# COMPiLELab/krylov_robustness

Measured on NVIDIA B200. Metric: krylov_matvecs_per_sec, higher is better.
Workload: dtype f64

## Files before the change

krylov_robustness_b200/csrc/api.cu:

```cuda
#include <memory>
#include <thread>
#include "common.cuh"
#include "csr.cuh"
#include "spmm.cuh"
#include "dense.cuh"
#include "slq.cuh"
#include "theta_table.h"
#include "smalldense.cuh"
#include "pairs.cuh"
#include "pairs_small.cuh"
#include "expmv.cuh"
#include "tsdense.cuh"
#include "smallgemm.cuh"
#include "vecops.cuh"
#include "blockkrylov.cuh"
#include "entries.cuh"
#include "entries_local.cuh"
#include "frechet.cuh"
#include "mctrace.cuh"
#include "nodepairs.cuh"

using namespace kr;

static void destroy_fun_update_result(kr_ctx* c);
// ... 15 lines not shown
        cudaError_t e = cudaGetDeviceCount(&count);
        if (e != cudaSuccess || count == 0) {
            cudaGetLastError();
            fail(KR_ERR_CUDA, "no CUDA device available (%s); this library has no CPU fallback",
                 e == cudaSuccess ? "device count is 0" : cudaGetErrorString(e));
        }
        if (device < 0 || device >= count) fail(KR_ERR_ARG, "device %d out of range (0..%d)", device, count - 1);
        KR_CUDA(cudaSetDevice(device));
        cudaDeviceProp prop;
        KR_CUDA(cudaGetDeviceProperties(&prop, device));
        if (prop.major < 10)
            fail(KR_ERR_CUDA, "device %d is sm_%d%d; this library is built for sm_100a only", device,
                 prop.major, prop.minor);
        kr_ctx* c = new kr_ctx();
        c->device = device;
        c->num_sms = prop.multiProcessorCount;
        c->l2_bytes = (size_t)prop.l2CacheSize;
        KR_CUDA(cudaStreamCreateWithFlags(&c->stream, cudaStreamNonBlocking));
        *out = c;
    });
}

void kr_ctx_destroy(kr_ctx* c) {
    if (!c) return;
    cudaSetDevice(c->device);
    cudaStreamSynchronize(c->stream);
    destroy_fun_update_result(c);
    for (auto& ev : c->spmm_events) {
        cudaEventDestroy(ev.first);
        cudaEventDestroy(ev.second);
    }
    for (auto ev : c->free_events) cudaEventDestroy(ev);
    c->trim();
    if (c->copy_stream) cudaStreamDestroy(c->copy_stream);
    if (c->stream) cudaStreamDestroy(c->stream);
    delete c;
}

int kr_ctx_sync(kr_ctx* c) {
    return guarded([&] {
        KR_CUDA(cudaSetDevice(c->device));
        KR_CUDA(cudaStreamSynchronize(c->stream));
    });
}

int kr_ctx_counters(kr_ctx* c, int64_t out[5]) {
    return guarded([&] {
        for (int i = 0; i < 5; ++i) out[i] = c->counters[i];
    });
}

int kr_ctx_set_timing(kr_ctx* c, int on) {
    return guarded([&] { c->timing = on != 0; });
}

int kr_ctx_spmm_time(kr_ctx* c, int reset, double* ms, int64_t* launches) {
    return guarded([&] {
        KR_CUDA(cudaStreamSynchronize(c->stream));
        for (auto& ev : c->spmm_events) {
            float t = 0.f;
            KR_CUDA(cudaEventElapsedTime(&t, ev.first, ev.second));
            c->spmm_ms += t;
            c->spmm_timed += 1;
            c->free_events.push_back(ev.first);
            c->free_events.push_back(ev.second);
        }
        c->spmm_events.clear();
        if (ms) *ms = c->spmm_ms;
        if (launches) *launches = c->spmm_timed;
        if (reset) {
            c->spmm_ms = 0.0;
            c->spmm_timed = 0;
        }
    });
}

void* kr_ctx_stream(kr_ctx* c) { return c ? (void*)c->stream : nullptr; }

int kr_matrix_create(kr_ctx* ctx, int64_t n, int64_t nnz, const int64_t* row_ptr, const int64_t* col_idx,
                     const double* val, kr_matrix** out) {
    return guarded([&] {
        if (!ctx || !out || !row_ptr || (nnz > 0 && (!col_idx || !val)))
            fail(KR_ERR_ARG, "kr_matrix_create: null argument");
        if (n < 0 || nnz < 0 || row_ptr[0] != 0 || row_ptr[n] != nnz)
            fail(KR_ERR_ARG, "kr_matrix_create: inconsistent row_ptr (the matrix A should be square, CSR, 0-based)");
        KR_CUDA(cudaSetDevice(ctx->device));
        std::unique_ptr<kr_matrix> M(new kr_matrix());
        M->ctx = ctx;
        M->host.n = n;
        M->host.row_ptr.assign(row_ptr, row_ptr + n + 1);
        M->host.col.resize(nnz);
        M->host.val.resize(nnz);
        for (int64_t i = 0; i < n; ++i)
            if (row_ptr[i + 1] < row_ptr[i]) fail(KR_ERR_ARG, "kr_matrix_create: row_ptr not monotone");
        int bad = 0;
#pragma omp parallel for reduction(|| : bad) schedule(static)
        for (int64_t p = 0; p < nnz; ++p) {
            bad = bad || col_idx[p] < 0 || col_idx[p] >= n;
            M->host.col[p] = (int32_t)col_idx[p];
            M->host.val[p] = val[p];
        }
        if (bad) fail(KR_ERR_ARG, "kr_matrix_create: column index out of range (The matrix A should be square)");
        analyse_and_upload(M.get());
        *out = M.release();
        if (const char* e = getenv("KR_GPUS")) {
            const int want = atoi(e);
            if (want > 1 && kr_matrix_replicate(*out, want, nullptr) != 0) {
                const std::string m = kr_last_error();
                kr_matrix_destroy(*out);
                *out = nullptr;
                fail(KR_ERR_CUDA, "KR_GPUS=%d: %s", want, m.c_str());
            }
        }
    });
}

void kr_matrix_destroy(kr_matrix* A) {
    if (!A) return;
    for (kr_matrix* P : A->peers) {
        kr_ctx* pc = P->ctx;
        cudaSetDevice(pc->device);
        delete P;
        kr_ctx_destroy(pc);
    }
    A->peers.clear();
    cudaSetDevice(A->ctx->device);
    delete A;
}

int kr_matrix_replicate(kr_matrix* A, int ndev, const int* devices) {
    return guarded([&] {
        if (!A || A->is_peer) fail(KR_ERR_ARG, "kr_matrix_replicate: null matrix or a replica");
        if (!A->peers.empty()) fail(KR_ERR_ARG, "kr_matrix_replicate: the matrix already has replicas");
        int count = 0;
        KR_CUDA(cudaGetDeviceCount(&count));
        std::vector<int> devs;
        if (ndev <= 0 || !devices) {
            const int want = ndev <= 0 ? count : std::min(ndev, count);
            for (int d = 0; d < count && (int)devs.size() < want - 1; ++d)
                if (d != A->ctx->device) devs.push_back(d);
        } else {
            for (int k = 0; k < ndev; ++k) {
                if (devices[k] < 0 || devices[k] >= count) fail(KR_ERR_ARG, "kr_matrix_replicate: device %d out of range", devices[k]);
                if (devices[k] != A->ctx->device) devs.push_back(devices[k]);
            }
        }
        materialize(A);
        const CsrHost& H = A->host;
        std::vector<int> status(devs.size(), 0);
        std::vector<std::string> msg(devs.size());
        std::vector<kr_matrix*> made(devs.size(), nullptr);
        std::vector<std::thread> th;
        for (size_t k = 0; k < devs.size(); ++k)
            th.emplace_back([&, k] {
                status[k] = guarded([&] {
                    kr_ctx* pc = nullptr;
                    if (kr_ctx_create(devs[k], &pc) != 0) fail(KR_ERR_CUDA, "%s", kr_last_error());
                    std::unique_ptr<kr_matrix> M(new kr_matrix());
                    M->ctx = pc;
                    M->host = H;
                    M->is_peer = true;
                    try { analyse_and_upload(M.get()); } catch (...) { M.reset(); kr_ctx_destroy(pc); throw; }
                    made[k] = M.release();
                });
                if (status[k]) msg[k] = kr_last_error();
            });
        for (auto& t : th) t.join();
        for (size_t k = 0; k < devs.size(); ++k)
            if (status[k]) {
                for (kr_matrix* P : made)
                    if (P) { kr_ctx* pc = P->ctx; cudaSetDevice(pc->device); delete P; kr_ctx_destroy(pc); }
                fail(status[k], "%s", msg[k].c_str());
            }
        A->peers = made;
        KR_CUDA(cudaSetDevice(A->ctx->device));
    });
}

int kr_matrix_replicas(const kr_matrix* A) { return A ? 1 + (int)A->peers.size() : 0; }

int kr_matrix_info(const kr_matrix* A, int64_t* n, int64_t* nnz, int* symmetric, int* pattern_only,
                   int* nonnegative) {
    return guarded([&] {
        if (!A) fail(KR_ERR_ARG, "null matrix");
        if (n) *n = A->dev.n;
        if (nnz) *nnz = A->dev.nnz;
        if (symmetric) *symmetric = A->symmetric;
        if (pattern_only) *pattern_only = A->dev.pattern_only;
        if (nonnegative) *nonnegative = A->nonnegative;
    });
}

int kr_matrix_set_edges(kr_matrix* A, int64_t count, const int64_t* ii, const int64_t* jj, const double* v) {
    return guarded([&] {
        if (!A) fail(KR_ERR_ARG, "null matrix");
        KR_CUDA(cudaSetDevice(A->ctx->device));
        const CsrHost& H = A->host;
        const int64_t n = H.n;
        for (int64_t e = 0; e < count; ++e) {
            const int64_t i = ii[e] - 1, j = jj[e] - 1;
            if (i < 0 || i >= n || j < 0 || j >= n) fail(KR_ERR_ARG, "kr_matrix_set_edges: index out of range");
            A->pending[{i, j}] = v[e] - host_entry(H, i, j);
            A->pending[{j, i}] = v[e] - host_entry(H, j, i);
        }
        for (auto it = A->pending.begin(); it != A->pending.end();)
            it = (it->second == 0.0) ? A->pending.erase(it) : std::next(it);
        if (!A->symmetric || A->pending.size() > KR_MAX_PENDING) flush_pending(A);
        else upload_pending(A);
        for (kr_matrix* P : A->peers)
            if (kr_matrix_set_edges(P, count, ii, jj, v) != 0) fail(KR_ERR_CUDA, "replica on device %d: %s", P->ctx->device, kr_last_error());
        KR_CUDA(cudaSetDevice(A->ctx->device));
    });
}

int kr_dense_create(kr_ctx* ctx, int64_t n, int64_t k, kr_dense** out) {
    return guarded([&] {
        if (!ctx || !out || n < 0 || k < 0 || k > (1 << 20)) fail(KR_ERR_ARG, "kr_dense_create: bad argument");
        KR_CUDA(cudaSetDevice(ctx->device));
        std::unique_ptr<kr_dense> d(new kr_dense());
        d->ctx = ctx;
        d->buf.reset(ctx, n, (int)k);
        *out = d.release();
    });
}

void kr_dense_destroy(kr_dense* d) {
    if (!d) return;
    cudaSetDevice(d->ctx->device);
    delete d;
}

static void upload_cm(kr_ctx* ctx, const double* host, int64_t ld, PanelBuf& dst) { upload_cm_block(ctx, host, ld, dst); }
static void download_cm(kr_ctx* ctx, const PanelBuf& src, double* host, int64_t ld) { download_cm_block(ctx, src, host, ld); }

int kr_dense_upload(kr_dense* d, const double* host, int64_t ld) {
    return guarded([&] {
        if (!d || !host) fail(KR_ERR_ARG, "kr_dense_upload: null argument");
        KR_CUDA(cudaSetDevice(d->ctx->device));
        upload_cm(d->ctx, host, ld, d->buf);
    });
}

int kr_dense_download(const kr_dense* d, double* host, int64_t ld) {
    return guarded([&] {
        if (!d || !host) fail(KR_ERR_ARG, "kr_dense_download: null argument");
        KR_CUDA(cudaSetDevice(d->ctx->device));
        download_cm(d->ctx, d->buf, host, ld);
    });
}

int kr_dense_fill_rademacher(kr_dense* d, uint64_t seed, int64_t col_offset) {
    return guarded([&] {
        if (!d) fail(KR_ERR_ARG, "null block");
        KR_CUDA(cudaSetDevice(d->ctx->device));
        if (d->buf.elems() == 0) return;
        KR_LAUNCH(d->ctx, rademacher_kernel, d->ctx->num_sms * 8, 256, 0, d->buf.p(), d->buf.n, d->buf.cols,
                  d->buf.panels, seed, col_offset);
    });
}

int kr_spmm_dev(kr_ctx* ctx, const kr_matrix* A, const kr_dense* X, kr_dense* Y) {
    return guarded([&] {
        if (!ctx || !A || !X || !Y) fail(KR_ERR_ARG, "kr_spmm_dev: null argument");
        if (X->buf.n != A->dev.n) fail(KR_ERR_ARG, "The block vector b has wrong number of rows");
        if (Y->buf.n != X->buf.n || Y->buf.cols != X->buf.cols || Y->buf.p() == X->buf.p())
            fail(KR_ERR_ARG, "kr_spmm_dev: Y must be a distinct block of the same shape as X");
        KR_CUDA(cudaSetDevice(ctx->device));
        EpiPlain epi{Y->buf.p(), X->buf.p(), 1.0, 0.0};
        launch_spmm(ctx, A->dev, X->buf.p(), X->buf.panels, epi, nullptr, X->buf.cols);
    });
}

int kr_spmm(kr_ctx* ctx, const kr_matrix* A, int64_t k, const double* X, int64_t ldx, double* Y, int64_t ldy) {
    return guarded([&] {
        if (!ctx || !A || !X || !Y) fail(KR_ERR_ARG, "kr_spmm: null argument");
        KR_CUDA(cudaSetDevice(ctx->device));
        const int64_t n = A->dev.n;
        PanelBuf xb(ctx, n, (int)k), yb(ctx, n, (int)k);
        upload_cm(ctx, X, ldx, xb);
        EpiPlain epi{yb.p(), xb.p(), 1.0, 0.0};
        launch_spmm(ctx, A->dev, xb.p(), xb.panels, epi, nullptr, (int)k);
        download_cm(ctx, yb, Y, ldy);
    });
}

static void slq_finish(const SlqResult& R, int64_t m, double* tr, double* vals, double* alpha, double* beta) {
    if (tr) *tr = R.tr;
    const size_t k = R.vals.size();
    if (vals) std::memcpy(vals, R.vals.data(), k * sizeof(double));
    if (alpha || beta)
        for (int64_t j = 0; j < m; ++j)
            for (size_t c = 0; c < k; ++c) {
                if (alpha) alpha[c * m + j] = R.alpha[(size_t)j * k + c];
                if (beta) beta[c * m + j] = R.beta[(size_t)j * k + c];
            }
}

int kr_slq_trace_dev(kr_ctx* ctx, const kr_matrix* A, const kr_dense* Z, int64_t m, int fun, double* tr,
                     double* vals, double* alpha, double* beta) {
    return guarded([&] {
        if (!ctx || !A || !Z) fail(KR_ERR_ARG, "kr_slq_trace_dev: null argument");
        if (fun < 0 || fun > 2) fail(KR_ERR_ARG, "unsupported function selector");
        KR_CUDA(cudaSetDevice(ctx->device));
        PanelBuf W(ctx, Z->buf.n, Z->buf.cols);
        KR_CUDA(cudaMemcpyAsync(W.p(), Z->buf.p(), (size_t)W.elems() * sizeof(double), cudaMemcpyDeviceToDevice,
                                ctx->stream));
        SlqResult R = slq_run(ctx, A, W, (int)m, fun, alpha || beta);
        slq_finish(R, m, tr, vals, alpha, beta);
    });
}

}

template <class T>
static int slq_trace_host(kr_ctx* ctx, const kr_matrix* A, int64_t k, const T* Z, int64_t ldz, int64_t m, int fun,
                          double* tr, double* vals, double* alpha, double* beta) {
    return guarded([&] {
        if (!ctx || !A || !Z) fail(KR_ERR_ARG, "kr_slq_trace: null argument");
        if (fun < 0 || fun > 2) fail(KR_ERR_ARG, "unsupported function selector");
        KR_CUDA(cudaSetDevice(ctx->device));
        const int64_t n = A->dev.n;
        if (ldz < n) fail(KR_ERR_ARG, "The block vector b has wrong number of rows");
        if (k <= 0) fail(KR_ERR_ARG, "kr_slq_trace: no probe columns");
        std::vector<int64_t> cstart, cwidth;
        for (int64_t c0 = 0; c0 < k;) {
            const int64_t cw = std::min<int64_t>(k - c0, cstart.empty() ? 2 * PW : (cstart.size() == 1 ? 6 * PW : 8 * PW));
            cstart.push_back(c0);
            cwidth.push_back(cw);
            c0 += cw;
        }
        if (cstart.empty()) { cstart.push_back(0); cwidth.push_back(0); }
        const int64_t nch = (int64_t)cstart.size();
        if (!ctx->copy_stream) KR_CUDA(cudaStreamCreateWithFlags(&ctx->copy_stream, cudaStreamNonBlocking));
        std::vector<std::unique_ptr<PanelBuf>> W(nch);
        std::vector<std::unique_ptr<DevBuf<T>>> stage(nch);
        std::vector<cudaEvent_t> ready(nch, nullptr);
        for (int64_t c = 0; c < nch; ++c) {
            W[c].reset(new PanelBuf(ctx, n, (int)cwidth[c]));
            stage[c].reset(new DevBuf<T>(ctx, (size_t)std::max<int64_t>(n * cwidth[c], 1)));
        }
        KR_CUDA(cudaStreamSynchronize(ctx->stream));
        auto issue_copy = [&](int64_t c) {
            const int64_t c0 = cstart[c], cw = cwidth[c];
            if (n > 0 && cw > 0) {
                KR_CUDA(cudaMemcpy2DAsync(stage[c]->p, n * sizeof(T), Z + c0 * ldz, ldz * sizeof(T),
                                          n * sizeof(T), cw, cudaMemcpyHostToDevice, ctx->copy_stream));
                ctx->counters[3] += n * cw * (int64_t)sizeof(T);
            }
            cm_to_panel(ctx, stage[c]->p, n, *W[c], ctx->copy_stream);
            KR_CUDA(cudaEventCreateWithFlags(&ready[c], cudaEventDisableTiming));
            KR_CUDA(cudaEventRecord(ready[c], ctx->copy_stream));
        };
        std::vector<double> all_vals((size_t)k), all_a, all_b;
        if (alpha || beta) { all_a.resize((size_t)m * k); all_b.resize((size_t)m * k); }
        auto harvest = [&](int64_t c, SlqJob& job) {
            const int64_t c0 = cstart[c], cw = cwidth[c];
            SlqResult R = job.collect();
            for (int64_t q = 0; q < cw; ++q) all_vals[(size_t)(c0 + q)] = R.vals[(size_t)q];
            if (alpha || beta)
                for (int64_t j = 0; j < m; ++j)
                    for (int64_t q = 0; q < cw; ++q) {
                        all_a[(size_t)(j * k + c0 + q)] = R.alpha[(size_t)(j * cw + q)];
                        all_b[(size_t)(j * k + c0 + q)] = R.beta[(size_t)(j * cw + q)];
                    }
        };
        try {
            issue_copy(0);
            std::unique_ptr<SlqJob> prev;
            for (int64_t c = 0; c < nch; ++c) {
                KR_CUDA(cudaStreamWaitEvent(ctx->stream, ready[c], 0));
                std::unique_ptr<SlqJob> job(new SlqJob(ctx, A, *W[c], (int)m, fun, alpha || beta));
                job->mark();
                if (c + 1 < nch) issue_copy(c + 1);
                if (prev) harvest(c - 1, *prev);
                prev = std::move(job);
            }
            if (prev) harvest(nch - 1, *prev);
        } catch (...) {
            cudaStreamSynchronize(ctx->copy_stream);
            cudaStreamSynchronize(ctx->stream);
            for (auto e : ready) if (e) cudaEventDestroy(e);
            throw;
        }
        KR_CUDA(cudaStreamSynchronize(ctx->copy_stream));
        for (auto e : ready) if (e) cudaEventDestroy(e);
        SlqResult R;
        R.vals = all_vals;
        R.alpha = all_a;
        R.beta = all_b;
        double s = 0.0;
        for (int64_t q = 0; q < k; ++q) s += all_vals[(size_t)q];
        R.tr = k ? s / (double)k : 0.0;
        slq_finish(R, m, tr, vals, alpha, beta);
    });
}

template <class T>
static int slq_trace_sharded(kr_ctx* ctx, const kr_matrix* A, int64_t k, const T* Z, int64_t ldz, int64_t m, int fun,
                             double* tr, double* vals, double* alpha, double* beta) {
    const int R = 1 + (int)A->peers.size();
    if (R == 1 || k < 2 * R || !Z) return slq_trace_host<T>(ctx, A, k, Z, ldz, m, fun, tr, vals, alpha, beta);
    std::vector<int> status(R, 0);
    std::vector<std::string> msg(R);
    std::vector<double> part(R, 0.0);
    std::vector<std::thread> th;
    for (int r = 0; r < R; ++r)
        th.emplace_back([&, r] {
            const int64_t lo = k * r / R, hi = k * (r + 1) / R;
            const kr_matrix* Ar = r == 0 ? A : A->peers[(size_t)r - 1];
            status[r] = slq_trace_host<T>(r == 0 ? ctx : Ar->ctx, Ar, hi - lo, Z + lo * ldz, ldz, m, fun, &part[r],
                                          vals ? vals + lo : nullptr, alpha ? alpha + lo * m : nullptr,
                                          beta ? beta + lo * m : nullptr);
            if (status[r]) msg[r] = kr_last_error();
        });
    for (auto& t : th) t.join();
    cudaSetDevice(ctx->device);
    for (int r = 0; r < R; ++r)
        if (status[r]) { tls_error() = msg[r]; return status[r]; }
    double s = 0.0;
    for (int r = 0; r < R; ++r) s += part[r] * (double)(k * (r + 1) / R - k * r / R);
    if (tr) *tr = s / (double)k;
    return KR_OK;
}

extern "C" {

int kr_slq_trace(kr_ctx* ctx, const kr_matrix* A, int64_t k, const double* Z, int64_t ldz, int64_t m, int fun,
                 double* tr, double* vals, double* alpha, double* beta) {
    if (!ctx || !A) { tls_error() = "kr_slq_trace: null argument"; return KR_ERR_ARG; }
    return slq_trace_sharded<double>(ctx, A, k, Z, ldz, m, fun, tr, vals, alpha, beta);
}

int kr_slq_trace_sign(kr_ctx* ctx, const kr_matrix* A, int64_t k, const signed char* Z, int64_t ldz, int64_t m, int fun,
                      double* tr, double* vals, double* alpha, double* beta) {
    if (!ctx || !A) { tls_error() = "kr_slq_trace: null argument"; return KR_ERR_ARG; }
    return slq_trace_sharded<signed char>(ctx, A, k, Z, ldz, m, fun, tr, vals, alpha, beta);
}

int kr_theta(double theta[100]) {
    return guarded([&] { std::memcpy(theta, KR_THETA, sizeof(KR_THETA)); });
}

}

#include "api_l2.inc"
```

krylov_robustness_b200/csrc/dense.cuh:

```cuda
#pragma once
#include "spmm.cuh"

namespace kr {

struct PanelBuf {
    DevBuf<double> buf;
    int64_t n = 0;
    int cols = 0, panels = 0;
    PanelBuf() = default;
    PanelBuf(kr_ctx* ctx, int64_t n_, int cols_) { reset(ctx, n_, cols_); }
    void reset(kr_ctx* ctx, int64_t n_, int cols_) {
        n = n_;
        cols = cols_;
        panels = (cols_ + PW - 1) / PW;
        buf.reset(ctx, (size_t)n * panels * PW);
    }
    double* p() const { return buf.p; }
    int64_t elems() const { return n * panels * PW; }
};

__global__ void __launch_bounds__(256)
cm_to_panel_kernel(const double* __restrict__ src, int64_t ld, int64_t n, int cols,
                   double* __restrict__ dst) {
    __shared__ double t[PW][65];
    const int q = blockIdx.y;
    const int64_t r0 = (int64_t)blockIdx.x * 64;
    for (int e = threadIdx.x; e < PW * 64; e += 256) {
        int c = e / 64, i = e % 64;
        int64_t r = r0 + i;
        int col = q * PW + c;
        t[c][i] = (r < n && col < cols) ? src[r + (int64_t)col * ld] : 0.0;
    }
    __syncthreads();
    double* d = dst + (int64_t)q * n * PW + r0 * PW;
    for (int e = threadIdx.x; e < PW * 64; e += 256) {
        int i = e / PW, c = e % PW;
        if (r0 + i < n) d[e] = t[c][i];
    }
}

__global__ void __launch_bounds__(256)
panel_to_cm_kernel(const double* __restrict__ src, int64_t n, int cols, double* __restrict__ dst,
                   int64_t ld) {
    __shared__ double t[PW][65];
    const int q = blockIdx.y;
    const int64_t r0 = (int64_t)blockIdx.x * 64;
    const double* s = src + (int64_t)q * n * PW + r0 * PW;
    for (int e = threadIdx.x; e < PW * 64; e += 256) {
        int i = e / PW, c = e % PW;
        t[c][i] = (r0 + i < n) ? s[e] : 0.0;
    }
    __syncthreads();
    for (int e = threadIdx.x; e < PW * 64; e += 256) {
        int c = e / 64, i = e % 64;
        int64_t r = r0 + i;
        int col = q * PW + c;
        if (r < n && col < cols) dst[r + (int64_t)col * ld] = t[c][i];
    }
}

__global__ void __launch_bounds__(256)
cm_i8_to_panel_kernel(const signed char* __restrict__ src, int64_t ld, int64_t n, int cols,
                      double* __restrict__ dst) {
    __shared__ signed char t[PW][64 + 4];
    const int q = blockIdx.y;
    const int64_t r0 = (int64_t)blockIdx.x * 64;
    for (int e = threadIdx.x; e < PW * 64; e += 256) {
        int c = e / 64, i = e % 64;
        int64_t r = r0 + i;
        int col = q * PW + c;
        t[c][i] = (r < n && col < cols) ? src[r + (int64_t)col * ld] : (signed char)0;
    }
    __syncthreads();
    double* d = dst + (int64_t)q * n * PW + r0 * PW;
    for (int e = threadIdx.x; e < PW * 64; e += 256) {
        int i = e / PW, c = e % PW;
        const int v = t[c][i];
        if (r0 + i < n) d[e] = v > 0 ? 1.0 : (v < 0 ? -1.0 : 0.0);
    }
}
inline void cm_to_panel(kr_ctx* ctx, const signed char* src_dev, int64_t ld, PanelBuf& dst, cudaStream_t stream = nullptr) {
    if (dst.n == 0 || dst.panels == 0) return;
    dim3 grid((unsigned)ceil_div(dst.n, 64), (unsigned)dst.panels);
    cm_i8_to_panel_kernel<<<grid, 256, 0, stream ? stream : ctx->stream>>>(src_dev, ld, dst.n, dst.cols, dst.p());
    check_launch(ctx, "cm_i8_to_panel_kernel");
}
inline void cm_to_panel(kr_ctx* ctx, const double* src_dev, int64_t ld, PanelBuf& dst, cudaStream_t stream = nullptr) {
    if (dst.n == 0 || dst.panels == 0) return;
    dim3 grid((unsigned)ceil_div(dst.n, 64), (unsigned)dst.panels);
    cm_to_panel_kernel<<<grid, 256, 0, stream ? stream : ctx->stream>>>(src_dev, ld, dst.n, dst.cols, dst.p());
    check_launch(ctx, "cm_to_panel_kernel");
}
inline void panel_to_cm(kr_ctx* ctx, const PanelBuf& src, double* dst_dev, int64_t ld) {
    if (src.n == 0 || src.panels == 0) return;
    dim3 grid((unsigned)ceil_div(src.n, 64), (unsigned)src.panels);
    KR_LAUNCH(ctx, panel_to_cm_kernel, grid, 256, 0, src.p(), src.n, src.cols, dst_dev, ld);
}

__host__ __device__ inline uint64_t splitmix64(uint64_t x) {
    x += 0x9E3779B97F4A7C15ull;
    x = (x ^ (x >> 30)) * 0xBF58476D1CE4E5B9ull;
    x = (x ^ (x >> 27)) * 0x94D049BB133111EBull;
    return x ^ (x >> 31);
}
__global__ void rademacher_kernel(double* __restrict__ dst, int64_t n, int cols, int panels,
                                  uint64_t seed, int64_t col_offset) {
    const int64_t total = n * panels * PW;
    for (int64_t e = (int64_t)blockIdx.x * blockDim.x + threadIdx.x; e < total;
         e += (int64_t)gridDim.x * blockDim.x) {
        int64_t q = e / (n * PW), rem = e % (n * PW);
        int64_t i = rem / PW;
        int c = (int)(q * PW + rem % PW);
        double v = 0.0;
        if (c < cols) {
            uint64_t h = splitmix64(seed ^ (((uint64_t)(c + col_offset) << 32) | (uint64_t)i));
            v = (h >> 63) ? -1.0 : 1.0;
        }
        dst[e] = v;
    }
}

constexpr int COL_THREADS = 256;
constexpr int COL_ROWS_PER_CTA = 2048;

inline int col_row_blocks(int64_t n) { return (int)ceil_div(n, COL_ROWS_PER_CTA); }

template <int NV>
__device__ __forceinline__ void col_cta_reduce(double (&v)[NV], double* smem) {
    cta_reduce_by_sub<NV>(v, smem);
}

__global__ void __launch_bounds__(COL_THREADS)
colnorm2_kernel(const double* __restrict__ X, int64_t n, double* __restrict__ partial, int total_cols) {
    __shared__ double smem[COL_WARPS * LPT * 2];
    const int q = blockIdx.y, sub = threadIdx.x % LPT;
    const double* Xp = X + (int64_t)q * n * PW;
    const int64_t r0 = (int64_t)blockIdx.x * COL_ROWS_PER_CTA;
    const int64_t r1 = min(n, r0 + COL_ROWS_PER_CTA);
    double acc[2] = {0.0, 0.0};
    for (int64_t r = r0 + (threadIdx.x / LPT); r < r1; r += COL_THREADS / LPT) {
        double2 x = *reinterpret_cast<const double2*>(Xp + r * PW + sub * 2);
        acc[0] += x.x * x.x;
        acc[1] += x.y * x.y;
    }
    col_cta_reduce<2>(acc, smem);
    if (threadIdx.x < LPT) {
        double* o = partial + (int64_t)blockIdx.x * total_cols + q * PW + threadIdx.x * 2;
        o[0] = acc[0];
        o[1] = acc[1];
    }
}

__global__ void __launch_bounds__(COL_THREADS)
combine3_norm_kernel(const double* __restrict__ Y, const double* __restrict__ U1,
                     const double* U0, double* W, int64_t n, const double* __restrict__ coef,
                     int total_cols, double* __restrict__ partial) {
    __shared__ double smem[COL_WARPS * LPT * 2];
    const int q = blockIdx.y, sub = threadIdx.x % LPT;
    const int64_t po = (int64_t)q * n * PW;
    const int col = q * PW + sub * 2;
    const double c0x = coef[col], c0y = coef[col + 1];
    const double c1x = coef[total_cols + col], c1y = coef[total_cols + col + 1];
    const double c2x = coef[2 * total_cols + col], c2y = coef[2 * total_cols + col + 1];
    const int64_t r0 = (int64_t)blockIdx.x * COL_ROWS_PER_CTA;
    const int64_t r1 = min(n, r0 + COL_ROWS_PER_CTA);
    double acc[2] = {0.0, 0.0};
    for (int64_t r = r0 + (threadIdx.x / LPT); r < r1; r += COL_THREADS / LPT) {
        const int64_t o = po + r * PW + sub * 2;
        double2 y = __ldcs(reinterpret_cast<const double2*>(Y + o));
        double2 u1 = *reinterpret_cast<const double2*>(U1 + o);
        double2 u0 = *reinterpret_cast<const double2*>(U0 + o);
        double2 w;
        w.x = c0x * y.x + c1x * u1.x + c2x * u0.x;
        w.y = c0y * y.y + c1y * u1.y + c2y * u0.y;
        *reinterpret_cast<double2*>(W + o) = w;
        acc[0] += w.x * w.x;
        acc[1] += w.y * w.y;
    }
    col_cta_reduce<2>(acc, smem);
    if (threadIdx.x < LPT) {
        double* o = partial + (int64_t)blockIdx.x * total_cols + q * PW + threadIdx.x * 2;
        o[0] = acc[0];
        o[1] = acc[1];
    }
}

__global__ void __launch_bounds__(256)
sum_partials_kernel(const double* __restrict__ partial, int nblocks, int total_cols,
                    double* __restrict__ out) {
    __shared__ double sm[8][33];
    const int tx = threadIdx.x & 31, ty = threadIdx.x >> 5;
    const int c = blockIdx.x * 32 + tx;
    double s = 0.0;
    if (c < total_cols)
        for (int b = ty; b < nblocks; b += 8) s += partial[(int64_t)b * total_cols + c];
    sm[ty][tx] = s;
    __syncthreads();
    if (ty == 0 && c < total_cols) {
        double t = 0.0;
#pragma unroll
        for (int k = 0; k < 8; ++k) t += sm[k][tx];
        out[c] = t;
    }
}

inline void sum_partials(kr_ctx* ctx, const double* partial, int nblocks, int total_cols, double* out) {
    KR_LAUNCH(ctx, sum_partials_kernel, (int)ceil_div(total_cols, 32), 256, 0, partial, nblocks, total_cols, out);
}

struct SlqState {
    double* s1;
    double* s0;
    double* beta_prev;
    double* coef;
    double* alpha;
    double* beta;
};

__global__ void slq_alpha_kernel(const double* __restrict__ sums, int total_cols, SlqState st, int j) {
    int c = blockIdx.x * blockDim.x + threadIdx.x;
    if (c >= total_cols) return;
    const double d = sums[c];
    const double s1 = st.s1[c];
    const double a = s1 * s1 * d;
    st.alpha[(int64_t)j * total_cols + c] = a;
    st.coef[c] = s1;
    st.coef[total_cols + c] = -a * s1;
    st.coef[2 * total_cols + c] = -st.beta_prev[c] * st.s0[c];
}

__global__ void slq_beta_kernel(const double* __restrict__ sums, int total_cols, SlqState st, int j) {
    int c = blockIdx.x * blockDim.x + threadIdx.x;
    if (c >= total_cols) return;
    const double d = sums[c];
    const double b = sqrt(d);
    st.beta[(int64_t)j * total_cols + c] = b;
    st.s0[c] = st.s1[c];
    st.s1[c] = (b > 0.0) ? 1.0 / b : 0.0;
    st.beta_prev[c] = b;
}

__global__ void slq_init_kernel(const double* __restrict__ sums, int total_cols, SlqState st,
                                double* __restrict__ nrm2) {
    int c = blockIdx.x * blockDim.x + threadIdx.x;
    if (c >= total_cols) return;
    const double d = sums[c];
    nrm2[c] = d;
    st.s1[c] = d > 0.0 ? 1.0 / sqrt(d) : 0.0;
    st.s0[c] = 0.0;
    st.beta_prev[c] = 0.0;
}

__device__ __forceinline__ double apply_fun(int fun, double x) {
    return fun == KR_FUN_EXP ? exp(x) : fun == KR_FUN_SINH ? sinh(x) : cosh(x);
}

constexpr int SLQ_MAX_M = 128;
__global__ void slq_quadrature_kernel(const double* __restrict__ alpha, const double* __restrict__ beta,
                                      const double* __restrict__ nrm2, int m, int cols, int total_cols,
                                      int fun, double* __restrict__ vals) {
    int c = blockIdx.x * blockDim.x + threadIdx.x;
    if (c >= cols) return;
    double d[SLQ_MAX_M], e[SLQ_MAX_M], z[SLQ_MAX_M];
    int n = m;
    for (int i = 0; i < m; ++i) {
        d[i] = alpha[(int64_t)i * total_cols + c];
        e[i] = beta[(int64_t)i * total_cols + c];
        z[i] = 0.0;
        if (n == m && !(e[i] > 0.0)) n = i + 1;
    }
    e[n - 1] = 0.0;
    z[0] = 1.0;
    for (int l = 0; l < n; ++l) {
        int iter = 0, mm;
        do {
            for (mm = l; mm < n - 1; ++mm) {
                double dd = fabs(d[mm]) + fabs(d[mm + 1]);
                if (fabs(e[mm]) <= 2.220446049250313e-16 * dd) break;
            }
            if (mm != l) {
                if (iter++ == 100) break;
                double g = (d[l + 1] - d[l]) / (2.0 * e[l]);
                double r = hypot(g, 1.0);
                g = d[mm] - d[l] + e[l] / (g + copysign(r, g));
                double s = 1.0, cc = 1.0, p = 0.0;
                int i;
                for (i = mm - 1; i >= l; --i) {
                    double f = s * e[i], b = cc * e[i];
                    r = hypot(f, g);
                    e[i + 1] = r;
                    if (r == 0.0) {
                        d[i + 1] -= p;
                        e[mm] = 0.0;
                        break;
                    }
                    s = f / r;
                    cc = g / r;
                    g = d[i + 1] - p;
                    r = (d[i] - g) * s + 2.0 * cc * b;
                    p = s * r;
                    d[i + 1] = g + p;
                    g = cc * r - b;
                    f = z[i + 1];
                    z[i + 1] = s * z[i] + cc * f;
                    z[i] = cc * z[i] - s * f;
                }
                if (r == 0.0 && i >= l) continue;
                d[l] -= p;
                e[l] = g;
                e[mm] = 0.0;
            }
        } while (mm != l);
    }
    double acc = 0.0;
    for (int i = 0; i < n; ++i) acc += z[i] * z[i] * apply_fun(fun, d[i]);
    vals[c] = nrm2[c] * acc;
}

}
```

krylov_robustness_b200/csrc/slq.cuh:

```cuda
#pragma once
#include "dense.cuh"

namespace kr {

struct SlqResult {
    double tr = 0.0;
    std::vector<double> vals, alpha, beta;
};

struct SlqJob {
    kr_ctx* ctx;
    int m, cols, tc;
    bool want_ab;
    PanelBuf B2, Y;
    DevBuf<double> partial, sums, scal, alpha, beta, vals;

    SlqJob(kr_ctx* c, const kr_matrix* M, PanelBuf& Z, int m_, int fun, bool want_ab_) : ctx(c), m(m_), want_ab(want_ab_) {
        if (m < 1 || m > SLQ_MAX_M) fail(KR_ERR_ARG, "slq: m must be in 1..%d", SLQ_MAX_M);
        const CsrDev& A = M->dev;
        const int64_t n = A.n;
        if (Z.n != n) fail(KR_ERR_ARG, "The block vector b has wrong number of rows");
        cols = Z.cols;
        const int panels = Z.panels;
        tc = panels * PW;
        B2.reset(ctx, n, cols);
        Y.reset(ctx, n, cols);
        B2.buf.zero();
        const int rb = col_row_blocks(n);
        const int nparts = std::max(rb, A.ntiles);
        partial.reset(ctx, (size_t)nparts * tc);
        sums.reset(ctx, tc);
        scal.reset(ctx, (size_t)tc * 7);
        alpha.reset(ctx, (size_t)m * tc);
        beta.reset(ctx, (size_t)m * tc);
        vals.reset(ctx, tc);
        scal.zero();
        SlqState st;
        st.s1 = scal.p;
        st.s0 = scal.p + tc;
        st.beta_prev = scal.p + 2 * tc;
        st.coef = scal.p + 3 * tc;
        double* nrm2 = scal.p + 6 * tc;
        st.alpha = alpha.p;
        st.beta = beta.p;
        const int sb = (int)ceil_div(tc, 128);
        dim3 cgrid((unsigned)rb, (unsigned)panels);
        KR_LAUNCH(ctx, colnorm2_kernel, cgrid, COL_THREADS, 0, Z.p(), n, partial.p, tc);
        sum_partials(ctx, partial.p, rb, tc, sums.p);
        KR_LAUNCH(ctx, slq_init_kernel, sb, 128, 0, sums.p, tc, st, nrm2);
        double* U1 = Z.p();
        double* U0 = B2.p();
        for (int j = 0; j < m; ++j) {
            EpiDot epi;
            epi.Y = Y.p();
            epi.X = U1;
            epi.partial = partial.p;
            epi.total_cols = tc;
            launch_spmm(ctx, A, U1, panels, epi, nullptr, cols);
            sum_partials(ctx, partial.p, A.ntiles, tc, sums.p);
            KR_LAUNCH(ctx, slq_alpha_kernel, sb, 128, 0, sums.p, tc, st, j);
            KR_LAUNCH(ctx, combine3_norm_kernel, cgrid, COL_THREADS, 0, Y.p(), U1, U0, U0, n, st.coef, tc, partial.p);
            sum_partials(ctx, partial.p, rb, tc, sums.p);
            KR_LAUNCH(ctx, slq_beta_kernel, sb, 128, 0, sums.p, tc, st, j);
            std::swap(U0, U1);
        }
        KR_LAUNCH(ctx, slq_quadrature_kernel, (int)ceil_div(cols, 64), 64, 0, alpha.p, beta.p, nrm2, m, cols, tc, fun, vals.p);
    }

    cudaEvent_t finished = nullptr;
    void mark() {
        KR_CUDA(cudaEventCreateWithFlags(&finished, cudaEventDisableTiming));
        KR_CUDA(cudaEventRecord(finished, ctx->stream));
    }
    ~SlqJob() { if (finished) cudaEventDestroy(finished); }

    SlqResult collect() {
        SlqResult R;
        std::vector<double> v(vals.count);
        if (finished) {
            KR_CUDA(cudaEventSynchronize(finished));
            cudaStream_t cs = ctx->copy_stream ? ctx->copy_stream : ctx->stream;
            KR_CUDA(cudaMemcpyAsync(v.data(), vals.p, v.size() * sizeof(double), cudaMemcpyDeviceToHost, cs));
            KR_CUDA(cudaStreamSynchronize(cs));
            ctx->counters[4] += (int64_t)(v.size() * sizeof(double));
        } else {
            v = vals.to_host();
        }
        R.vals.assign(v.begin(), v.begin() + cols);
        double s = 0.0;
        for (int c = 0; c < cols; ++c) s += R.vals[c];
        R.tr = cols ? s / cols : 0.0;
        if (want_ab) {
            if (finished) KR_CUDA(cudaStreamSynchronize(ctx->stream));
            std::vector<double> a = alpha.to_host(), b = beta.to_host();
            R.alpha.resize((size_t)m * cols);
            R.beta.resize((size_t)m * cols);
            for (int j = 0; j < m; ++j)
                for (int c = 0; c < cols; ++c) {
                    R.alpha[(size_t)j * cols + c] = a[(size_t)j * tc + c];
                    R.beta[(size_t)j * cols + c] = b[(size_t)j * tc + c];
                }
        }
        return R;
    }
};

inline SlqResult slq_run(kr_ctx* ctx, const kr_matrix* M, PanelBuf& Z, int m, int fun, bool want_ab) {
    SlqJob job(ctx, M, Z, m, fun, want_ab);
    return job.collect();
}

}
```

krylov_robustness_b200/csrc/spmm.cuh:

```cuda
#pragma once
#include "csr.cuh"

namespace kr {

#ifndef KR_PW
#define KR_PW 16
#endif
constexpr int PW = KR_PW;
constexpr int LPT = PW / 2;
static_assert(PW == 8 || PW == 16, "panel width must be 8 or 16");
#ifndef KR_SPMM_THREADS
#define KR_SPMM_THREADS 256
#endif
constexpr int SPMM_THREADS = KR_SPMM_THREADS;
constexpr int COL_WARPS = 8;
constexpr int SPMM_WARPS = SPMM_THREADS / 32;
#ifndef KR_SPMM_MIN_CTAS
#define KR_SPMM_MIN_CTAS 4
#endif
constexpr int SPMM_MIN_CTAS = KR_SPMM_MIN_CTAS;

struct PanelBlock {
    double* p;
    int64_t n;
    int cols;
    int panels;
    __host__ __device__ double* panel(int q) const { return p + (int64_t)q * n * PW; }
};

template <int CPL>
struct Vec {
    double v[CPL];
};
template <int CPL>
__device__ __forceinline__ Vec<CPL> vzero() {
    Vec<CPL> r;
#pragma unroll
    for (int i = 0; i < CPL; ++i) r.v[i] = 0.0;
    return r;
}
template <int CPL>
__device__ __forceinline__ Vec<CPL> ld_x(const double* p);
template <>
__device__ __forceinline__ Vec<2> ld_x<2>(const double* p) {
    const double2 t = __ldg(reinterpret_cast<const double2*>(p));
    Vec<2> r;
    r.v[0] = t.x; r.v[1] = t.y;
    return r;
}
template <>
__device__ __forceinline__ Vec<4> ld_x<4>(const double* p) {
    Vec<4> r;
    asm("ld.global.nc.v4.f64 {%0, %1, %2, %3}, [%4];"
        : "=d"(r.v[0]), "=d"(r.v[1]), "=d"(r.v[2]), "=d"(r.v[3]) : "l"(p));
    return r;
}
__device__ __forceinline__ Vec<4> ld_row(const double* p) {
    Vec<4> r;
    asm volatile("ld.global.v4.f64 {%0, %1, %2, %3}, [%4];"
                 : "=d"(r.v[0]), "=d"(r.v[1]), "=d"(r.v[2]), "=d"(r.v[3]) : "l"(p));
    return r;
}
__device__ __forceinline__ void st_row(double* p, const Vec<4>& a) {
    asm volatile("st.global.v4.f64 [%0], {%1, %2, %3, %4};" ::"l"(p), "d"(a.v[0]), "d"(a.v[1]), "d"(a.v[2]), "d"(a.v[3]) : "memory");
}
__device__ __forceinline__ void st_stream(double* p, const Vec<4>& a) {
    asm volatile("st.global.cs.v4.f64 [%0], {%1, %2, %3, %4};" ::"l"(p), "d"(a.v[0]), "d"(a.v[1]), "d"(a.v[2]), "d"(a.v[3]) : "memory");
}
#ifndef KR_SPMM_PF
#define KR_SPMM_PF 1
#endif
__device__ __forceinline__ void prefetch_x(const double* p) {
    asm volatile("prefetch.global.L2 [%0];" ::"l"(p));
}
__device__ __forceinline__ void prefetch_l1(const double* p) {
    asm volatile("prefetch.global.L1 [%0];" ::"l"(p));
}
__device__ __forceinline__ int ld_stream(const int* p) { return __ldcs(p); }
__device__ __forceinline__ double ld_stream(const double* p) { return __ldcs(p); }
__device__ __forceinline__ void st_stream(double* p, double2 v) {
    __stcs(reinterpret_cast<double2*>(p), v);
}

template <int NV, int WARPS = COL_WARPS, int LP = LPT>
__device__ __forceinline__ void cta_reduce_by_sub(double (&v)[NV], double* smem) {
    const int lane = threadIdx.x & 31, warp = threadIdx.x >> 5;
#pragma unroll
    for (int i = 0; i < NV; ++i) {
        double x = v[i];
#pragma unroll
        for (int off = LP; off < 32; off <<= 1) x += __shfl_xor_sync(0xffffffffu, x, off);
        v[i] = x;
    }
    if (lane < LP) {
#pragma unroll
        for (int i = 0; i < NV; ++i) smem[(warp * LP + lane) * NV + i] = v[i];
    }
    __syncthreads();
    if (warp == 0 && lane < LP) {
#pragma unroll
        for (int i = 0; i < NV; ++i) {
            double s = 0.0;
            for (int w = 0; w < WARPS; ++w) s += smem[(w * LP + lane) * NV + i];
            v[i] = s;
        }
    }
}


struct EpiPlain {
    static constexpr int CPL = 4;
    double* __restrict__ Y;
    const double* __restrict__ X;
    double alpha, mu;
    __device__ __forceinline__ void init(int q, int64_t stride) {
        Y += q * stride;
        X += q * stride;
    }
    Vec<CPL> xr;
    __device__ __forceinline__ void pre(int r, int sub) {
        if (mu != 0.0 && sub == 0) prefetch_l1(X + (int64_t)r * PW);
    }
    __device__ __forceinline__ void row(int r, int sub, Vec<CPL> y, unsigned) {
        if (mu != 0.0) xr = ld_row(X + (int64_t)r * PW + sub * CPL);
#pragma unroll
        for (int i = 0; i < CPL; ++i) {
            if (mu != 0.0) y.v[i] -= mu * xr.v[i];
            y.v[i] *= alpha;
        }
        st_stream(Y + (int64_t)r * PW + sub * CPL, y);
    }
    __device__ __forceinline__ void finish(int, int, double*) {}
};

struct EpiDot {
    static constexpr int CPL = 4;
    double* __restrict__ Y;
    const double* __restrict__ X;
    double* __restrict__ partial;
    int total_cols;
    double acc[CPL];
    __device__ __forceinline__ void init(int q, int64_t stride) {
        Y += q * stride;
        X += q * stride;
#pragma unroll
        for (int i = 0; i < CPL; ++i) acc[i] = 0.0;
    }
    Vec<CPL> xr;
    __device__ __forceinline__ void pre(int r, int sub) {
        if (sub == 0) prefetch_l1(X + (int64_t)r * PW);
    }
    __device__ __forceinline__ void row(int r, int sub, Vec<CPL> y, unsigned) {
        xr = ld_row(X + (int64_t)r * PW + sub * CPL);
#pragma unroll
        for (int i = 0; i < CPL; ++i) acc[i] += xr.v[i] * y.v[i];
        st_stream(Y + (int64_t)r * PW + sub * CPL, y);
    }
    __device__ __forceinline__ void finish(int tile, int panel, double* smem) {
        cta_reduce_by_sub<CPL, SPMM_WARPS, PW / CPL>(acc, smem);
        if (threadIdx.x < PW / CPL) {
            double* o = partial + (int64_t)tile * total_cols + panel * PW + threadIdx.x * CPL;
#pragma unroll
            for (int i = 0; i < CPL; ++i) o[i] = acc[i];
        }
    }
};

struct EpiGram2 {
    static constexpr int CPL = 2;
    double* __restrict__ Y;
    const double* __restrict__ P;
    const double* __restrict__ C;
    double* __restrict__ partial;
    int ncand;
    double acc[8];
    __device__ __forceinline__ void init(int q, int64_t stride) {
        Y += q * stride;
        C += q * stride;
        if (P) P += q * stride;
#pragma unroll
        for (int i = 0; i < 8; ++i) acc[i] = 0.0;
    }
    __device__ __forceinline__ void pre(int r, int sub) {
        if (sub == 0) {
            prefetch_l1(C + (int64_t)r * PW);
            if (P) prefetch_l1(P + (int64_t)r * PW);
        }
    }
    __device__ __forceinline__ void row(int r, int sub, Vec<2> yv, unsigned) {
        const int64_t o = (int64_t)r * PW + sub * 2;
        const double2 y = make_double2(yv.v[0], yv.v[1]);
        const double2 c = *reinterpret_cast<const double2*>(C + o);
        if (P) {
            const double2 p = *reinterpret_cast<const double2*>(P + o);
            acc[0] += p.x * y.x; acc[1] += p.x * y.y;
            acc[2] += p.y * y.x; acc[3] += p.y * y.y;
        }
        acc[4] += c.x * y.x; acc[5] += c.x * y.y;
        acc[6] += c.y * y.x; acc[7] += c.y * y.y;
        st_stream(Y + o, y);
    }
    __device__ __forceinline__ void finish(int tile, int panel, double* smem) {
        cta_reduce_by_sub<8, SPMM_WARPS>(acc, smem);
        if (threadIdx.x < LPT) {
            double* o = partial + ((int64_t)tile * ncand + panel * LPT + threadIdx.x) * 8;
#pragma unroll
            for (int i = 0; i < 8; ++i) o[i] = acc[i];
        }
    }
};

struct TaylorCtl {
    double c1;
    double c2, nf;
    int done;
    int mv;
    unsigned long long mb_bits, mf_bits;
    unsigned int ticket;
};

__device__ __forceinline__ void taylor_decide(TaylorCtl* ctl, double c2, double nf, int full_term, double tol) {
    ctl->mv += 1;
    ctl->c2 = c2;
    ctl->nf = nf;
    if (!full_term) {
        if (ctl->c1 + c2 <= tol * nf) ctl->done = 1;
        else ctl->c1 = c2;
    }
}

struct EpiTaylor {
    static constexpr int CPL = 4;
    double* __restrict__ Bn;
    const double* __restrict__ Bo;
    double* __restrict__ F;
    double* __restrict__ rab;
    double* __restrict__ raf;
    double coef, mu;
    TaylorCtl* ctl;
    int total_ctas, full_term;
    double tol;
    double mb, mf;
    __device__ __forceinline__ void init(int q, int64_t stride) {
        Bn += q * stride;
        Bo += q * stride;
        F += q * stride;
        if (!ctl) {
            rab += q * (stride / PW);
            raf += q * (stride / PW);
        }
        mb = mf = 0.0;
    }
    Vec<CPL> xr, fr;
    __device__ __forceinline__ void pre(int r, int sub) {
        if (sub == 0) {
            if (mu != 0.0) prefetch_l1(Bo + (int64_t)r * PW);
            prefetch_l1(F + (int64_t)r * PW);
        }
    }
    __device__ __forceinline__ void row(int r, int sub, Vec<CPL> y, unsigned m) {
        const int64_t o = (int64_t)r * PW + sub * CPL;
        if (mu != 0.0) xr = ld_row(Bo + o);
        fr = ld_row(F + o);
        Vec<CPL> f = fr;
        double ab = 0.0, af = 0.0;
#pragma unroll
        for (int i = 0; i < CPL; ++i) {
            if (mu != 0.0) y.v[i] -= mu * xr.v[i];
            y.v[i] *= coef;
            f.v[i] += y.v[i];
            ab += fabs(y.v[i]);
            af += fabs(f.v[i]);
        }
        st_row(F + o, f);
        st_stream(Bn + o, y);
#pragma unroll
        for (int off = 1; off < PW / CPL; off <<= 1) {
            ab += __shfl_xor_sync(m, ab, off);
            af += __shfl_xor_sync(m, af, off);
        }
        if (ctl) {
            mb = fmax(mb, ab);
            mf = fmax(mf, af);
        } else if (sub == 0) {
            rab[r] = ab;
            raf[r] = af;
        }
    }
    __device__ __forceinline__ void finish(int, int, double* smem) {
        if (!ctl) return;
        double a = mb, b = mf;
        for (int off = 16; off; off >>= 1) {
            a = fmax(a, __shfl_xor_sync(0xffffffffu, a, off));
            b = fmax(b, __shfl_xor_sync(0xffffffffu, b, off));
        }
        const int lane = threadIdx.x & 31, warp = threadIdx.x >> 5;
        if (lane == 0) { smem[2 * warp] = a; smem[2 * warp + 1] = b; }
        __syncthreads();
        if (threadIdx.x == 0) {
            for (int w = 1; w < SPMM_WARPS; ++w) { a = fmax(a, smem[2 * w]); b = fmax(b, smem[2 * w + 1]); }
            atomicMax(&ctl->mb_bits, (unsigned long long)__double_as_longlong(a));
            atomicMax(&ctl->mf_bits, (unsigned long long)__double_as_longlong(b));
            __threadfence();
            const unsigned t = atomicAdd(&ctl->ticket, 1u);
            if (t == (unsigned)total_ctas - 1u) {
                __threadfence();
                const double c2 = __longlong_as_double((long long)atomicAdd(&ctl->mb_bits, 0ull));
                const double nf = __longlong_as_double((long long)atomicAdd(&ctl->mf_bits, 0ull));
                taylor_decide(ctl, c2, nf, full_term, tol);
                ctl->mb_bits = 0ull;
                ctl->mf_bits = 0ull;
                ctl->ticket = 0u;
                __threadfence();
            }
        }
    }
};

constexpr size_t SPMM_SMEM_PATTERN = SPMM_CAP * sizeof(int) + (SPMM_MAX_ROWS + 1 + SPMM_MAX_ROWS + 3) * sizeof(int);
constexpr size_t SPMM_SMEM_VALUED = SPMM_SMEM_PATTERN + SPMM_CAP * sizeof(double);

template <bool HAS_VAL, int U, int CPL, bool PRED>
__device__ __forceinline__ void gather_block(int p, int p_end, int stride, const int* __restrict__ scol,
                                             const double* __restrict__ sval, const double* __restrict__ xs,
                                             Vec<CPL>& acc0, Vec<CPL>& acc1) {
    Vec<CPL> x[U];
    double v[U];
#pragma unroll
    for (int u = 0; u < U; ++u) {
        const int q = p + u * stride;
        if (PRED) {
            x[u] = vzero<CPL>();
            v[u] = 1.0;
        }
        if (!PRED || q < p_end) {
            x[u] = ld_x<CPL>(xs + (int64_t)scol[q] * PW);
            if (HAS_VAL) v[u] = sval[q];
        }
    }
#pragma unroll
    for (int u = 0; u < U; ++u) {
#pragma unroll
        for (int i = 0; i < CPL; ++i) {
            const bool second = (u & 1) && CPL == 2;
            if (HAS_VAL) {
                if (second) acc1.v[i] = fma(v[u], x[u].v[i], acc1.v[i]);
                else acc0.v[i] = fma(v[u], x[u].v[i], acc0.v[i]);
            } else {
                if (second) acc1.v[i] += x[u].v[i];
                else acc0.v[i] += x[u].v[i];
            }
        }
    }
}

template <bool HAS_VAL, int U, int CPL>
__device__ __forceinline__ Vec<CPL> gather_accumulate(int p_first, int p_end, int stride, const int* __restrict__ scol,
                                                      const double* __restrict__ sval, const double* __restrict__ xs,
                                                      const double* __restrict__ xpanel, int pf_sub) {
    Vec<CPL> acc0 = vzero<CPL>(), acc1 = vzero<CPL>();
    int p = p_first;
    for (; p + (U - 1) * stride < p_end; p += U * stride) {
#if KR_SPMM_PF > 0
        if (CPL == 2) {
            const int qpf = p + (KR_SPMM_PF * U + pf_sub) * stride;
            if (pf_sub < U && qpf < p_end) prefetch_x(xpanel + (int64_t)scol[qpf] * PW);
        }
#endif
        gather_block<HAS_VAL, U, CPL, false>(p, p_end, stride, scol, sval, xs, acc0, acc1);
    }
    if (p < p_end) gather_block<HAS_VAL, U, CPL, true>(p, p_end, stride, scol, sval, xs, acc0, acc1);
    if (CPL == 2) {
#pragma unroll
        for (int i = 0; i < CPL; ++i) acc0.v[i] += acc1.v[i];
    }
    return acc0;
}

template <int L, bool HAS_VAL, int U, bool DELTA, class Epi>
__device__ __forceinline__ void spmm_tile(const RowTile t, const int* __restrict__ srp, const int* __restrict__ srid,
                                          const int* __restrict__ scol, const double* __restrict__ sval,
                                          const double* __restrict__ Xp, double uval, Epi& epi, const CsrDevView& A,
                                          int e0, int e1) {
    constexpr int CPL = Epi::CPL;
    constexpr int LP = PW / CPL;
    constexpr int S = L / LP;
    constexpr int RPW = 32 / L;
    const int lane = threadIdx.x & 31, warp = threadIdx.x >> 5;
    const int sub = lane % LP;
    const int slot = (lane % L) / LP;
    const int rlocal = lane / L;
    const double* xs = Xp + sub * CPL;
    for (int base = warp * RPW; base < t.count; base += SPMM_WARPS * RPW) {
        const int rr = base + rlocal;
        const bool valid = rr < t.count;
        int row = 0, p0 = 0, p1 = 0;
        if (valid) {
            row = srid[rr];
            p0 = srp[rr];
            p1 = srp[rr + 1];
        }
        const bool emit = valid && slot == 0;
        if (emit) epi.pre(row, sub);
#if KR_SPMM_PF > 0
        if (CPL == 2) {
            const int rn = rr + KR_SPMM_PF * SPMM_WARPS * RPW;
            if (rn < t.count) {
                const int q0 = srp[rn], q1 = srp[rn + 1];
#pragma unroll
                for (int k = 0; k < KR_SPMM_PF; ++k) {
                    const int q = q0 + slot + (k * U + sub) * S;
                    if (sub < U && q < q1) prefetch_x(Xp + (int64_t)scol[q] * PW);
                }
            }
        }
#endif
        Vec<CPL> acc = gather_accumulate<HAS_VAL, U, CPL>(p0 + slot, p1, S, scol, sval, xs, Xp, sub);
#pragma unroll
        for (int off = LP; off < L; off <<= 1) {
#pragma unroll
            for (int i = 0; i < CPL; ++i) acc.v[i] += __shfl_xor_sync(0xffffffffu, acc.v[i], off);
        }
        if (!HAS_VAL) {
#pragma unroll
            for (int i = 0; i < CPL; ++i) acc.v[i] *= uval;
        }
        if (DELTA && e1 > e0 && emit) {
            for (int e = e0; e < e1; ++e)
                if (A.dl_rowlocal[e] == rr) {
                    const Vec<CPL> x = ld_x<CPL>(xs + (int64_t)A.dl_col[e] * PW);
                    const double d = A.dl_val[e];
#pragma unroll
                    for (int i = 0; i < CPL; ++i) acc.v[i] = fma(d, x.v[i], acc.v[i]);
                }
        }
        const unsigned m = __ballot_sync(0xffffffffu, emit);
        if (emit) epi.row(row, sub, acc, m);
    }
}

template <class Epi, bool HAS_VAL, int U, bool DELTA>
__device__ __forceinline__ void spmm_item(const CsrDevView& A, const double* __restrict__ X, const Epi& epi_proto,
                                          int64_t panel_stride, int tile, int panel, double* red, unsigned char* dyn_smem) {
    constexpr int CPL = Epi::CPL;
    constexpr int LP = PW / CPL;
    int* scol = reinterpret_cast<int*>(dyn_smem);
    int* srp = scol + SPMM_CAP;
    int* srid = srp + SPMM_MAX_ROWS + 1;
    double* sval = reinterpret_cast<double*>(dyn_smem + SPMM_SMEM_PATTERN);
    const RowTile t = A.tiles[tile];
    const int pb = __ldg(A.row_ptr + t.start);
    const int nz = __ldg(A.row_ptr + t.start + t.count) - pb;
    const bool long_row = t.lanes_log2 == 6;
    const int e0 = DELTA && A.dl_tile_begin ? A.dl_tile_begin[tile] : 0;
    const int e1 = DELTA && A.dl_tile_begin ? A.dl_tile_begin[tile + 1] : 0;
    Epi epi = epi_proto;
    epi.init(panel, panel_stride);
    const double* Xp = X + (int64_t)panel * panel_stride;
    if (!long_row) {
        for (int i = threadIdx.x; i <= t.count; i += SPMM_THREADS) srp[i] = __ldg(A.row_ptr + t.start + i) - pb;
        for (int i = threadIdx.x; i < t.count; i += SPMM_THREADS) srid[i] = __ldg(A.row_order + t.start + i);
        for (int p = threadIdx.x; p < nz; p += SPMM_THREADS) scol[p] = ld_stream(A.col + pb + p);
        if (HAS_VAL)
            for (int p = threadIdx.x; p < nz; p += SPMM_THREADS) sval[p] = ld_stream(A.val + pb + p);
        __syncthreads();
        switch (t.lanes_log2) {
            case 0: spmm_tile<LP, HAS_VAL, U, DELTA>(t, srp, srid, scol, sval, Xp, A.uval, epi, A, e0, e1); break;
            case 1: spmm_tile<2 * LP, HAS_VAL, U, DELTA>(t, srp, srid, scol, sval, Xp, A.uval, epi, A, e0, e1); break;
            case 2: spmm_tile<(4 * LP > 32 ? 32 : 4 * LP), HAS_VAL, U, DELTA>(t, srp, srid, scol, sval, Xp, A.uval, epi, A, e0, e1); break;
// ... 108 lines not shown
```

Before: 49410.

## Avoid probe copy and skip redundant SLQ Lanczos traffic

The SLQ driver no longer copies the probe block into a scratch buffer. It now rotates three work buffers so the input stays read-only. The first combine step skips reading the zero U0 vector, and the final Lanczos step uses a dot-only SpMM epilogue that does not store Y and skips the last combine and normalisation. The partial-sum reduction loop is also unrolled to issue more loads at once. The cost is one extra panel buffer, plus a quadrature change that zeroes the last beta, which is needed because the final beta is no longer computed.

```diff
diff --git a/krylov_robustness_b200/csrc/api.cu b/krylov_robustness_b200/csrc/api.cu
--- a/krylov_robustness_b200/csrc/api.cu
+++ b/krylov_robustness_b200/csrc/api.cu
@@ -341,10 +341,7 @@
         if (!ctx || !A || !Z) fail(KR_ERR_ARG, "kr_slq_trace_dev: null argument");
         if (fun < 0 || fun > 2) fail(KR_ERR_ARG, "unsupported function selector");
         KR_CUDA(cudaSetDevice(ctx->device));
-        PanelBuf W(ctx, Z->buf.n, Z->buf.cols);
-        KR_CUDA(cudaMemcpyAsync(W.p(), Z->buf.p(), (size_t)W.elems() * sizeof(double), cudaMemcpyDeviceToDevice,
-                                ctx->stream));
-        SlqResult R = slq_run(ctx, A, W, (int)m, fun, alpha || beta);
+        SlqResult R = slq_run(ctx, A, Z->buf, (int)m, fun, alpha || beta);
         slq_finish(R, m, tr, vals, alpha, beta);
     });
 }
diff --git a/krylov_robustness_b200/csrc/dense.cuh b/krylov_robustness_b200/csrc/dense.cuh
--- a/krylov_robustness_b200/csrc/dense.cuh
+++ b/krylov_robustness_b200/csrc/dense.cuh
@@ -151,6 +151,7 @@
     }
 }
 
+template <bool FIRST>
 __global__ void __launch_bounds__(COL_THREADS)
 combine3_norm_kernel(const double* __restrict__ Y, const double* __restrict__ U1,
                      const double* U0, double* W, int64_t n, const double* __restrict__ coef,
@@ -169,10 +170,14 @@
         const int64_t o = po + r * PW + sub * 2;
         double2 y = __ldcs(reinterpret_cast<const double2*>(Y + o));
         double2 u1 = *reinterpret_cast<const double2*>(U1 + o);
-        double2 u0 = *reinterpret_cast<const double2*>(U0 + o);
         double2 w;
-        w.x = c0x * y.x + c1x * u1.x + c2x * u0.x;
-        w.y = c0y * y.y + c1y * u1.y + c2y * u0.y;
+        w.x = c0x * y.x + c1x * u1.x;
+        w.y = c0y * y.y + c1y * u1.y;
+        if (!FIRST) {
+            double2 u0 = *reinterpret_cast<const double2*>(U0 + o);
+            w.x = w.x + c2x * u0.x;
+            w.y = w.y + c2y * u0.y;
+        }
         *reinterpret_cast<double2*>(W + o) = w;
         acc[0] += w.x * w.x;
         acc[1] += w.y * w.y;
@@ -192,8 +197,18 @@
     const int tx = threadIdx.x & 31, ty = threadIdx.x >> 5;
     const int c = blockIdx.x * 32 + tx;
     double s = 0.0;
-    if (c < total_cols)
-        for (int b = ty; b < nblocks; b += 8) s += partial[(int64_t)b * total_cols + c];
+    if (c < total_cols) {
+        constexpr int B = 16;
+        int b = ty;
+        for (; b + 8 * (B - 1) < nblocks; b += 8 * B) {
+            double v[B];
+#pragma unroll
+            for (int k = 0; k < B; ++k) v[k] = partial[(int64_t)(b + 8 * k) * total_cols + c];
+#pragma unroll
+            for (int k = 0; k < B; ++k) s += v[k];
+        }
+        for (; b < nblocks; b += 8) s += partial[(int64_t)b * total_cols + c];
+    }
     sm[ty][tx] = s;
     __syncthreads();
     if (ty == 0 && c < total_cols) {
@@ -265,7 +280,7 @@
     int n = m;
     for (int i = 0; i < m; ++i) {
         d[i] = alpha[(int64_t)i * total_cols + c];
-        e[i] = beta[(int64_t)i * total_cols + c];
+        e[i] = i + 1 < m ? beta[(int64_t)i * total_cols + c] : 0.0;
         z[i] = 0.0;
         if (n == m && !(e[i] > 0.0)) n = i + 1;
     }
diff --git a/krylov_robustness_b200/csrc/slq.cuh b/krylov_robustness_b200/csrc/slq.cuh
--- a/krylov_robustness_b200/csrc/slq.cuh
+++ b/krylov_robustness_b200/csrc/slq.cuh
@@ -12,10 +12,10 @@
     kr_ctx* ctx;
     int m, cols, tc;
     bool want_ab;
-    PanelBuf B2, Y;
+    PanelBuf W0, W1, Y;
     DevBuf<double> partial, sums, scal, alpha, beta, vals;
 
-    SlqJob(kr_ctx* c, const kr_matrix* M, PanelBuf& Z, int m_, int fun, bool want_ab_) : ctx(c), m(m_), want_ab(want_ab_) {
+    SlqJob(kr_ctx* c, const kr_matrix* M, const PanelBuf& Z, int m_, int fun, bool want_ab_) : ctx(c), m(m_), want_ab(want_ab_) {
         if (m < 1 || m > SLQ_MAX_M) fail(KR_ERR_ARG, "slq: m must be in 1..%d", SLQ_MAX_M);
         const CsrDev& A = M->dev;
         const int64_t n = A.n;
@@ -23,9 +23,9 @@
         cols = Z.cols;
         const int panels = Z.panels;
         tc = panels * PW;
-        B2.reset(ctx, n, cols);
+        W0.reset(ctx, n, cols);
+        if (m > 1) W1.reset(ctx, n, cols);
         Y.reset(ctx, n, cols);
-        B2.buf.zero();
         const int rb = col_row_blocks(n);
         const int nparts = std::max(rb, A.ntiles);
         partial.reset(ctx, (size_t)nparts * tc);
@@ -48,21 +48,36 @@
         KR_LAUNCH(ctx, colnorm2_kernel, cgrid, COL_THREADS, 0, Z.p(), n, partial.p, tc);
         sum_partials(ctx, partial.p, rb, tc, sums.p);
         KR_LAUNCH(ctx, slq_init_kernel, sb, 128, 0, sums.p, tc, st, nrm2);
-        double* U1 = Z.p();
-        double* U0 = B2.p();
+        const double* U1 = Z.p();
+        const double* U0 = nullptr;
+        double* W = W0.p();
         for (int j = 0; j < m; ++j) {
-            EpiDot epi;
-            epi.Y = Y.p();
-            epi.X = U1;
-            epi.partial = partial.p;
-            epi.total_cols = tc;
-            launch_spmm(ctx, A, U1, panels, epi, nullptr, cols);
+            const bool dot_only = j == m - 1 && !want_ab;
+            if (dot_only) {
+                EpiDotOnly epi;
+                epi.Y = nullptr;
+                epi.X = U1;
+                epi.partial = partial.p;
+                epi.total_cols = tc;
+                launch_spmm(ctx, A, U1, panels, epi, nullptr, cols);
+            } else {
+                EpiDot epi;
+                epi.Y = Y.p();
+                epi.X = U1;
+                epi.partial = partial.p;
+                epi.total_cols = tc;
+                launch_spmm(ctx, A, U1, panels, epi, nullptr, cols);
+            }
             sum_partials(ctx, partial.p, A.ntiles, tc, sums.p);
             KR_LAUNCH(ctx, slq_alpha_kernel, sb, 128, 0, sums.p, tc, st, j);
-            KR_LAUNCH(ctx, combine3_norm_kernel, cgrid, COL_THREADS, 0, Y.p(), U1, U0, U0, n, st.coef, tc, partial.p);
+            if (dot_only) break;
+            if (j == 0) KR_LAUNCH(ctx, combine3_norm_kernel<true>, cgrid, COL_THREADS, 0, Y.p(), U1, U0, W, n, st.coef, tc, partial.p);
+            else KR_LAUNCH(ctx, combine3_norm_kernel<false>, cgrid, COL_THREADS, 0, Y.p(), U1, U0, W, n, st.coef, tc, partial.p);
             sum_partials(ctx, partial.p, rb, tc, sums.p);
             KR_LAUNCH(ctx, slq_beta_kernel, sb, 128, 0, sums.p, tc, st, j);
-            std::swap(U0, U1);
+            U0 = U1;
+            U1 = W;
+            W = j == 0 ? W1.p() : const_cast<double*>(U0);
         }
         KR_LAUNCH(ctx, slq_quadrature_kernel, (int)ceil_div(cols, 64), 64, 0, alpha.p, beta.p, nrm2, m, cols, tc, fun, vals.p);
     }
@@ -105,7 +120,7 @@
     }
 };
 
-inline SlqResult slq_run(kr_ctx* ctx, const kr_matrix* M, PanelBuf& Z, int m, int fun, bool want_ab) {
+inline SlqResult slq_run(kr_ctx* ctx, const kr_matrix* M, const PanelBuf& Z, int m, int fun, bool want_ab) {
     SlqJob job(ctx, M, Z, m, fun, want_ab);
     return job.collect();
 }
diff --git a/krylov_robustness_b200/csrc/spmm.cuh b/krylov_robustness_b200/csrc/spmm.cuh
--- a/krylov_robustness_b200/csrc/spmm.cuh
+++ b/krylov_robustness_b200/csrc/spmm.cuh
@@ -133,7 +133,8 @@
     __device__ __forceinline__ void finish(int, int, double*) {}
 };
 
-struct EpiDot {
+template <bool STORE>
+struct EpiDotT {
     static constexpr int CPL = 4;
     double* __restrict__ Y;
     const double* __restrict__ X;
@@ -141,7 +142,7 @@
     int total_cols;
     double acc[CPL];
     __device__ __forceinline__ void init(int q, int64_t stride) {
-        Y += q * stride;
+        if (STORE) Y += q * stride;
         X += q * stride;
 #pragma unroll
         for (int i = 0; i < CPL; ++i) acc[i] = 0.0;
@@ -154,7 +155,7 @@
         xr = ld_row(X + (int64_t)r * PW + sub * CPL);
 #pragma unroll
         for (int i = 0; i < CPL; ++i) acc[i] += xr.v[i] * y.v[i];
-        st_stream(Y + (int64_t)r * PW + sub * CPL, y);
+        if (STORE) st_stream(Y + (int64_t)r * PW + sub * CPL, y);
     }
     __device__ __forceinline__ void finish(int tile, int panel, double* smem) {
         cta_reduce_by_sub<CPL, SPMM_WARPS, PW / CPL>(acc, smem);
@@ -165,6 +166,8 @@
         }
     }
 };
+using EpiDot = EpiDotT<true>;
+using EpiDotOnly = EpiDotT<false>;
 
 struct EpiGram2 {
     static constexpr int CPL = 2;
```

Measured after the change: 50600, median of 6. +2.4%, better.
